# 0215Arthur/Pytorch_News_Recommender

Measured on AMD Instinct MI355X. Metric: users/sec (train step) NRMS MIND-small hist=50 cand=5, higher is better.
Workload: dtype f16 (MFMA inputs and saved activations; fp32 accumulate, softmax, loss, master weights and Adam); 1 GPU; configs[1] shapes: NRMS(nrms_v0) train step, 512 users/GPU, hist=50, cand=5, title_len=30, d=300, h=10, q=200, V=45800, dropout=0.2, Adam(lr=1e-3); users_per_gpu=512, global_batch=512, parallelism=dp1, precision=fp16, resident_batches=32

## Files before the change

pytorch_news_recommender_amd/csrc/fused16.h:

```cpp
#pragma once
#include "gemm.h"

namespace nrms {

typedef _Float16 h8 __attribute__((ext_vector_type(8)));
typedef _Float16 h4 __attribute__((ext_vector_type(4)));
typedef _Float16 h2 __attribute__((ext_vector_type(2)));

__device__ __forceinline__ f32x16 mfma32h(const h8& a, const h8& b, const f32x16& c) {
    return __builtin_amdgcn_mfma_f32_32x32x16_f16(a, b, c, 0, 0, 0);
}

__device__ __forceinline__ h8 acc_frag(const f32x16& x, int s) {
    h8 r;
#pragma unroll
    for (int j = 0; j < 8; ++j) r[j] = (_Float16)x[8 * s + j];
    return r;
}

__device__ __forceinline__ int p16_pos(int fpad) {
    const int b = fpad >> 4, t = fpad & 15;
    const int hh = (t >> 2) & 1, j = ((t >> 3) << 2) | (t & 3);
    return 16 * b + 8 * hh + j;
}

#ifdef NRMS_F16_EXPERIMENTS
#define F16_DBG(flags, bit) ((flags) & (bit))
#else
#define F16_DBG(flags, bit) 0
#endif

constexpr int F16_WAVES = 4;
constexpr int F16_THREADS = 64 * F16_WAVES;
constexpr int F16_KS = 20;
constexpr int F16_CS = 20;
constexpr int F16_QT = 7;
constexpr int F16_KP = 16 * F16_KS, F16_DP = 16 * F16_CS, F16_QP = 32 * F16_QT;
constexpr int F16_PITCH = (F16_KP + 8) * 2;
constexpr int F16_SLOT = 32 * F16_PITCH;
constexpr int F16_RC = F16_KP / 8;
static_assert(F16_KP == F16_DP, "one tile geometry for the head tiles and the additive tiles");
constexpr int F16_STG = (32 * F16_RC + F16_THREADS - 1) / F16_THREADS;
constexpr bool F16_STG_EXACT = 32 * F16_RC == F16_STG * F16_THREADS;

__device__ __forceinline__ long frag_off(long seq_block, int c16, int s, int l32, int hh) {
    return (seq_block * c16 + s) * 512 + l32 * 16 + 8 * hh;
}

struct TileRing {
    char* smem;
    const _Float16* src;
    int n_tiles, tid, l32, hh;
    int dbg;
    h8 stg[F16_STG];
    __device__ __forceinline__ void load(int n) {
        if (n >= n_tiles) return;
        if (F16_DBG(dbg, 1)) return;
        const char* t = reinterpret_cast<const char*>(src) + (long)n * (32 * F16_KP * 2);
        const unsigned off = (unsigned)tid * 16u;
#pragma unroll
        for (int i = 0; i < F16_STG; ++i)
            if (F16_STG_EXACT || i + 1 < F16_STG || tid + F16_THREADS * i < 32 * F16_RC)
                stg[i] = *reinterpret_cast<const h8*>(t + (long)F16_THREADS * 16 * i + off);
    }
    __device__ __forceinline__ void store(int n) {
        if (n >= n_tiles) return;
        if (F16_DBG(dbg, 1)) return;
        char* dst = smem + (n % 3) * F16_SLOT;
#pragma unroll
        for (int i = 0; i < F16_STG; ++i) {
            const int c = tid + F16_THREADS * i;
            if (F16_STG_EXACT || i + 1 < F16_STG || c < 32 * F16_RC) {
                const int row = c / F16_RC, col = c - row * F16_RC;
                *reinterpret_cast<h8*>(dst + row * F16_PITCH + col * 16) = stg[i];
            }
        }
    }
    __device__ __forceinline__ h8 frag(int n, int s) const {
        return *reinterpret_cast<const h8*>(smem + (n % 3) * F16_SLOT + l32 * F16_PITCH + (16 * s + 8 * hh) * 2);
    }
};

constexpr int F16_SLOT_DMA = 32 * F16_KP * 2;
static_assert(F16_SLOT_DMA == 5 * F16_WAVES * 1024, "five 1-KiB DMA pieces per wave and tile");
template <int SLOTS>
struct TileRingDMA {
    static constexpr int AHEAD = SLOTS - 1;
    char* smem;
    const _Float16* src;
    int n_tiles, wave, lane, l32, hh;
    __device__ __forceinline__ void load(int n) {
        if (n >= n_tiles) return;
        const char* g = reinterpret_cast<const char*>(src) + (long)n * F16_SLOT_DMA + wave * 1024 + lane * 16;
        char* l = smem + (n % SLOTS) * F16_SLOT_DMA + wave * 1024;
#pragma unroll
        for (int i = 0; i < 5; ++i)
            __builtin_amdgcn_global_load_lds((const __attribute__((address_space(1))) void*)(g + i * (F16_WAVES * 1024)),
                                             (__attribute__((address_space(3))) void*)(l + i * (F16_WAVES * 1024)), 16, 0, 0);
    }
    __device__ __forceinline__ void load_piece(int n, int i) {
        if (n >= n_tiles) return;
        const char* g = reinterpret_cast<const char*>(src) + (long)n * F16_SLOT_DMA + wave * 1024 + lane * 16 + i * (F16_WAVES * 1024);
        char* l = smem + (n % SLOTS) * F16_SLOT_DMA + wave * 1024 + i * (F16_WAVES * 1024);
        __builtin_amdgcn_global_load_lds((const __attribute__((address_space(1))) void*)g, (__attribute__((address_space(3))) void*)l, 16, 0, 0);
    }
    __device__ __forceinline__ void load_group(int n, int g) {
        if (SLOTS == 3) { load_piece(n, g); return; }
        if (g == 0) { load_piece(n, 0); load_piece(n, 1); }
        if (g == 1) { load_piece(n, 2); load_piece(n, 3); }
        if (g == 2) load_piece(n, 4);
    }
    __device__ __forceinline__ void load_at(int step, int tile) {
        const char* g = reinterpret_cast<const char*>(src) + (long)tile * F16_SLOT_DMA + wave * 1024 + lane * 16;
        char* l = smem + (step % SLOTS) * F16_SLOT_DMA + wave * 1024;
#pragma unroll
        for (int i = 0; i < 5; ++i)
            __builtin_amdgcn_global_load_lds((const __attribute__((address_space(1))) void*)(g + i * (F16_WAVES * 1024)),
                                             (__attribute__((address_space(3))) void*)(l + i * (F16_WAVES * 1024)), 16, 0, 0);
    }
    __device__ __forceinline__ void load_piece_at(int step, int tile, int i) {
        const char* g = reinterpret_cast<const char*>(src) + (long)tile * F16_SLOT_DMA + wave * 1024 + lane * 16 + i * (F16_WAVES * 1024);
        char* l = smem + (step % SLOTS) * F16_SLOT_DMA + wave * 1024 + i * (F16_WAVES * 1024);
        __builtin_amdgcn_global_load_lds((const __attribute__((address_space(1))) void*)g, (__attribute__((address_space(3))) void*)l, 16, 0, 0);
    }
    __device__ __forceinline__ void store(int) {}
    template <int YOUNGER = 0>
    __device__ __forceinline__ void step_barrier(int n) {
        static_assert(YOUNGER == 0 || YOUNGER == 2 || YOUNGER == 4 || YOUNGER == 8, "add the immediate below");
        if (SLOTS == 3 && n + 2 < n_tiles) {
            if (YOUNGER == 0) __asm__ volatile("s_waitcnt vmcnt(5)" ::: "memory");
            if (YOUNGER == 2) __asm__ volatile("s_waitcnt vmcnt(7)" ::: "memory");
            if (YOUNGER == 4) __asm__ volatile("s_waitcnt vmcnt(9)" ::: "memory");
            if (YOUNGER == 8) __asm__ volatile("s_waitcnt vmcnt(13)" ::: "memory");
        } else {
            __asm__ volatile("s_waitcnt vmcnt(0)" ::: "memory");
        }
        __asm__ volatile("s_waitcnt lgkmcnt(0)\n\ts_barrier" ::: "memory");
    }
    __device__ __forceinline__ h8 frag(int n, int s) const {
        return *reinterpret_cast<const h8*>(smem + (n % SLOTS) * F16_SLOT_DMA + ((2 * s + hh) * 32 + l32) * 16);
    }
};
__host__ __device__ __forceinline__ int dma_tile_pos(int r, int k) { return (((k >> 4) * 2 + ((k >> 3) & 1)) * 32 + r) * 8 + (k & 7); }

struct NoPrefetch { __device__ __forceinline__ void operator()(int) const {} };
template <bool W_IS_A, class Ring, int NS, class Between = NoPrefetch>
__device__ __forceinline__ void tile_mma(f32x16& acc, const Ring& ring, int n, const h8 (&op)[NS], Between between = Between()) {
    static_assert(NS % 4 == 0, "k-steps in groups of 4");
    h8 wa[4], wb[4];
#pragma unroll
    for (int i = 0; i < 4; ++i) wa[i] = ring.frag(n, i);
#pragma unroll
    for (int g = 0; g < NS / 4; ++g) {
        if (g + 1 < NS / 4) {
#pragma unroll
            for (int i = 0; i < 4; ++i) {
                if (g & 1) wa[i] = ring.frag(n, 4 * (g + 1) + i);
                else wb[i] = ring.frag(n, 4 * (g + 1) + i);
            }
        }
#pragma unroll
        for (int i = 0; i < 4; ++i) {
            const h8& w = (g & 1) ? wb[i] : wa[i];
            acc = W_IS_A ? mfma32h(w, op[4 * g + i], acc) : mfma32h(op[4 * g + i], w, acc);
        }
        between(g);
        __builtin_amdgcn_sched_barrier(0);
    }
}

__device__ __forceinline__ f32x16 rows_of(const float* v, int hh) {
    f32x16 r;
#pragma unroll
    for (int g = 0; g < 4; ++g) {
        const f32x4 bb = *reinterpret_cast<const f32x4*>(v + 8 * g + 4 * hh);
#pragma unroll
        for (int e = 0; e < 4; ++e) r[4 * g + e] = bb[e];
    }
    return r;
}
__device__ __forceinline__ f32x16 zero16() {
    f32x16 r;
#pragma unroll
    for (int i = 0; i < 16; ++i) r[i] = 0.f;
    return r;
}


}
```

pytorch_news_recommender_amd/csrc/fused16.hip:

```cpp
#include <stdlib.h>

#include "fused16.h"

namespace nrms {

struct Fwd16Args {
    int n_seq, S, d, h, dk, q;
    const _Float16* x16;
    const int* pos;
    const int* n_rows;
    const int64_t* ids;
    const int* order;
    const int* order_cnt;
    const _Float16* wtiles;
    const float* bqkv32;
    const float* badd32;
    const float* qv32;
    _Float16* ctx16;
    _Float16* t16;
    float* w;
    float* out;
    Dropout drop;
    int dbg;
};

#ifndef F16_FWD_SLOTS
#define F16_FWD_SLOTS 3
#endif
constexpr int F16_FWD_WGS = F16_FWD_SLOTS == 2 ? 3 : 2;
template <bool TRAIN, int SB>
__global__ __launch_bounds__(F16_THREADS, SB == 1 ? F16_FWD_WGS : 1) void fused_fwd16_kernel(Fwd16Args a) {
    extern __shared__ __attribute__((aligned(16))) char smem[];
    const int tid = threadIdx.x, lane = tid & 63;
    const int wave = __builtin_amdgcn_readfirstlane(tid >> 6);
    const int l32 = lane & 31, hh = lane >> 5;
    const int S = a.S;
    constexpr int KP = F16_KP, DP = F16_DP;
    const int n_head_tiles = 3 * a.h;

    int slot_id = blockIdx.x * F16_WAVES + wave;
    bool valid = slot_id < a.n_seq;
    int seq = slot_id;
    if (a.order != nullptr) {
        const int n_ne = a.order_cnt[0], n_e = a.order_cnt[1];
        const int g_ne = (n_ne + F16_WAVES - 1) / F16_WAVES;
        if ((int)blockIdx.x < g_ne) { valid = slot_id < n_ne; seq = valid ? a.order[slot_id] : 0; }
        else {
            slot_id -= g_ne * F16_WAVES;
            valid = slot_id < n_e;
            seq = valid ? a.order[a.n_seq + slot_id] : 0;
        }
    }
    if (!valid) seq = 0;
    const long tok0 = (long)seq * S;
    bool tok_ok[SB];
#pragma unroll
    for (int b = 0; b < SB; ++b) tok_ok[b] = valid && 32 * b + l32 < S;
    bool empty = false;
    if (SB == 1 && a.ids != nullptr && valid) {
        const bool is_pad = lane < S ? a.ids[tok0 + lane] == 0 : true;
        empty = __ballot(is_pad) == ~0ull;
    }
    const bool live = valid && !empty;
    const bool skip_heads = __syncthreads_and(live ? 0 : 1) != 0;
    const int n_begin = skip_heads ? n_head_tiles : 0;

    using Ring = TileRingDMA<SB == 1 ? F16_FWD_SLOTS : 3>;
    constexpr int AH = Ring::AHEAD;
    Ring ring;
    ring.smem = smem; ring.src = a.wtiles; ring.n_tiles = n_head_tiles + F16_QT; ring.wave = wave; ring.lane = lane; ring.l32 = l32; ring.hh = hh;
#pragma unroll
    for (int i = 0; i < AH; ++i) ring.load(n_begin + i);
    float* addv = reinterpret_cast<float*>(smem + (SB == 1 ? F16_FWD_SLOTS : 3) * F16_SLOT_DMA);
    for (int i = tid; i < 2 * F16_QP; i += F16_THREADS) addv[i] = i < F16_QP ? a.badd32[i] : a.qv32[i - F16_QP];

    h8 xf[SB][F16_KS];
#pragma unroll
    for (int b = 0; b < SB; ++b) {
        long row = -1;
        if (tok_ok[b] && !empty) {
            row = a.pos != nullptr ? (long)a.pos[tok0 + 32 * b + l32] : tok0 + 32 * b + l32;
            if (row < 0) row = *a.n_rows;
        }
        const _Float16* xr = a.x16 + (row < 0 ? 0 : row) * KP + 8 * hh;
#pragma unroll
        for (int s = 0; s < F16_KS; ++s) xf[b][s] = *reinterpret_cast<const h8*>(xr + 16 * s);
        if (row < 0) {
#pragma unroll
            for (int s = 0; s < F16_KS; ++s) xf[b][s] = h8{0, 0, 0, 0, 0, 0, 0, 0};
        }
    }
    __builtin_amdgcn_s_waitcnt(0x0F70);
    __asm__ volatile("s_waitcnt lgkmcnt(0)\n\ts_barrier" ::: "memory");

    int n = n_begin;
#pragma unroll 1
    for (int head = 0; head < a.h; ++head) {
        f32x16 ct[SB];
        if (!skip_heads) {
            f32x16 qt[SB], kt[SB], vv[SB];
            auto pre = [&](int g) { ring.load_group(n + AH, g); };
            if (!live) ring.load(n + AH);
#pragma unroll
            for (int b = 0; b < SB; ++b) {
                qt[b] = zero16();
                if (live) { if (b == 0) tile_mma<true>(qt[b], ring, n, xf[b], pre); else tile_mma<true>(qt[b], ring, n, xf[b]); }
            }
            ring.step_barrier(n);
            ++n;
            if (!live) ring.load(n + AH);
#pragma unroll
            for (int b = 0; b < SB; ++b) {
                kt[b] = zero16();
                if (live) { if (b == 0) tile_mma<true>(kt[b], ring, n, xf[b], pre); else tile_mma<true>(kt[b], ring, n, xf[b]); }
            }
            ring.step_barrier(n);
            ++n;
            if (!live) ring.load(n + AH);
#pragma unroll
            for (int b = 0; b < SB; ++b) {
                vv[b] = zero16();
                if (live) { if (b == 0) tile_mma<false>(vv[b], ring, n, xf[b], pre); else tile_mma<false>(vv[b], ring, n, xf[b]); }
            }
            if (live) {
#pragma unroll
                for (int ib = 0; ib < SB; ++ib) {
                    f32x16 st[SB];
                    float m = -3.0e38f;
#pragma unroll
                    for (int jb = 0; jb < SB; ++jb) {
                        st[jb] = mfma32h(acc_frag(kt[jb], 0), acc_frag(qt[ib], 0), zero16());
                        st[jb] = mfma32h(acc_frag(kt[jb], 1), acc_frag(qt[ib], 1), st[jb]);
#pragma unroll
                        for (int r = 0; r < 16; ++r) {
                            st[jb][r] = 32 * jb + crow32(r, hh) < S ? st[jb][r] : -3.0e38f;
                            m = fmaxf(m, st[jb][r]);
                        }
                    }
                    m = fmaxf(m, __shfl_xor(m, 32, 64));
                    float sum = 0.f;
#pragma unroll
                    for (int jb = 0; jb < SB; ++jb)
#pragma unroll
                        for (int r = 0; r < 16; ++r) {
                            const float p = 32 * jb + crow32(r, hh) < S ? __expf(st[jb][r] - m) : 0.f;
                            st[jb][r] = p;
                            sum += p;
                        }
                    sum += __shfl_xor(sum, 32, 64);
                    const float inv = 1.0f / sum;
                    ct[ib] = zero16();
#pragma unroll
                    for (int jb = 0; jb < SB; ++jb) {
#pragma unroll
                        for (int r = 0; r < 16; ++r) st[jb][r] *= inv;
                        ct[ib] = mfma32h(acc_frag(vv[jb], 0), acc_frag(st[jb], 0), ct[ib]);
                        ct[ib] = mfma32h(acc_frag(vv[jb], 1), acc_frag(st[jb], 1), ct[ib]);
                    }
                }
            }
        }
        if (!live) {
#pragma unroll
            for (int b = 0; b < SB; ++b) ct[b] = rows_of(a.bqkv32 + (3 * head + 2) * 32, hh);
        }
#pragma unroll
        for (int b = 0; b < SB; ++b) {
            if (a.drop.thresh != 0u) {
#pragma unroll
                for (int c = 0; c < 2; ++c) {
                    const uint64_t e0 = (uint64_t)(tok0 + 32 * b + l32) * (uint64_t)DP + (uint64_t)(head * 32 + 16 * c + 8 * hh);
                    float sc[8];
                    dropout_scale8(a.drop.seed, 1u, e0 >> 3, a.drop.thresh16, a.drop.inv_keep, sc);
#pragma unroll
                    for (int e = 0; e < 8; ++e) ct[b][8 * c + e] *= sc[e];
                }
            }
            if (valid && !F16_DBG(a.dbg, 8)) {
                const h8 z = {0, 0, 0, 0, 0, 0, 0, 0};
                _Float16* dst = a.ctx16 + frag_off((long)seq * SB + b, F16_CS, 2 * head, l32, hh);
                *reinterpret_cast<h8*>(dst) = tok_ok[b] ? acc_frag(ct[b], 0) : z;
                *reinterpret_cast<h8*>(dst + 512) = tok_ok[b] ? acc_frag(ct[b], 1) : z;
            }
        }
        if (!skip_heads) {
            ring.step_barrier(n);
            ++n;
        }
    }
#pragma unroll
    for (int b = 0; b < SB; ++b) {
        if (valid) {
            for (int head = a.h; head < F16_CS / 2; ++head) {
                _Float16* dst = a.ctx16 + frag_off((long)seq * SB + b, F16_CS, 2 * head, l32, hh);
                *reinterpret_cast<h8*>(dst) = h8{0, 0, 0, 0, 0, 0, 0, 0};
                *reinterpret_cast<h8*>(dst + 512) = h8{0, 0, 0, 0, 0, 0, 0, 0};
            }
        }
    }

    __asm__ volatile("s_waitcnt vmcnt(0)" ::: "memory");
    h8 cf[SB][F16_CS];
#pragma unroll
    for (int b = 0; b < SB; ++b) {
        const _Float16* src = a.ctx16 + frag_off((long)seq * SB + b, F16_CS, 0, l32, hh);
#pragma unroll
        for (int s = 0; s < F16_CS; ++s) cf[b][s] = *reinterpret_cast<const h8*>(src + (F16_DBG(a.dbg, 16) ? 0 : 512 * s));
    }
    float score[SB];
#pragma unroll
    for (int b = 0; b < SB; ++b) score[b] = 0.f;
#pragma unroll 1
    for (int t = 0; t < F16_QT; ++t) {
        const f32x16 ba = rows_of(addv + 32 * t, hh), qq = rows_of(addv + F16_QP + 32 * t, hh);
        __builtin_amdgcn_sched_barrier(0);
        auto pre2 = [&](int g) { ring.load_group(n + AH, g); };
        if (!valid) ring.load(n + AH);
#pragma unroll
        for (int b = 0; b < SB; ++b) {
            f32x16 tt = zero16();
            if (valid) { if (b == 0) tile_mma<true>(tt, ring, n, cf[b], pre2); else tile_mma<true>(tt, ring, n, cf[b]); }
#pragma unroll
            for (int g = 0; g < 4; ++g) {
                h4 th;
#pragma unroll
                for (int e = 0; e < 4; ++e) {
                    const float ex = __builtin_amdgcn_exp2f(fmaf(tt[4 * g + e], 2.885390082f, ba[4 * g + e]));
                    const float v = fmaf(-2.0f, __builtin_amdgcn_rcpf(ex + 1.0f), 1.0f);
                    score[b] += qq[4 * g + e] * v;
                    th[e] = (_Float16)v;
                }
                if (TRAIN && valid && !F16_DBG(a.dbg, 4)) {
                    if (!tok_ok[b]) th = h4{0, 0, 0, 0};
                    *reinterpret_cast<h4*>(a.t16 + ((((long)seq * SB + b) * (F16_QP / 16) + 2 * t + (g >> 1)) * 32 + l32) * 16 +
                                           8 * (g & 1) + 4 * hh) = th;
                }
            }
        }
        ring.step_barrier(n);
        ++n;
    }
    float mx = -3.0e38f;
#pragma unroll
    for (int b = 0; b < SB; ++b) {
        score[b] += __shfl_xor(score[b], 32, 64);
        score[b] = 32 * b + l32 < S ? score[b] : -3.0e38f;
        mx = fmaxf(mx, score[b]);
    }
#pragma unroll
    for (int o = 16; o > 0; o >>= 1) mx = fmaxf(mx, __shfl_xor(mx, o, 64));
    float es = 0.f, wgt[SB];
#pragma unroll
    for (int b = 0; b < SB; ++b) {
        wgt[b] = 32 * b + l32 < S ? __expf(score[b] - mx) : 0.f;
        es += wgt[b];
    }
#pragma unroll
    for (int o = 16; o > 0; o >>= 1) es += __shfl_xor(es, o, 64);
#pragma unroll
    for (int b = 0; b < SB; ++b) {
        wgt[b] /= es;
        if (TRAIN && a.w != nullptr && tok_ok[b] && hh == 0) a.w[tok0 + 32 * b + l32] = wgt[b];
    }

    if (valid) {
        h8 sel[2];
#pragma unroll
        for (int s2 = 0; s2 < 2; ++s2)
#pragma unroll
            for (int j = 0; j < 8; ++j) sel[s2][j] = (_Float16)(l32 == 16 * s2 + 8 * hh + j ? 1.0f : 0.0f);
        float wrow[SB][16];
#pragma unroll
        for (int b = 0; b < SB; ++b)
#pragma unroll
            for (int r = 0; r < 16; ++r) wrow[b][r] = __shfl(wgt[b], crow32(r, hh), 64);
#pragma unroll
        for (int p = 0; p < F16_CS / 2; ++p) {
            float acc = 0.f;
#pragma unroll
            for (int b = 0; b < SB; ++b) {
                f32x16 dd = mfma32h(cf[b][2 * p], sel[0], zero16());
                dd = mfma32h(cf[b][2 * p + 1], sel[1], dd);
#pragma unroll
                for (int r = 0; r < 16; ++r) acc += wrow[b][r] * dd[r];
            }
            acc += __shfl_xor(acc, 32, 64);
            const int n = l32, f = 16 * (n >> 4) + 8 * ((n & 7) >> 2) + 4 * ((n >> 3) & 1) + (n & 3);
            if (hh == 0 && f < a.dk && p < a.h) a.out[(long)seq * a.d + p * a.dk + f] = acc;
        }
    }
}

template <bool TRAIN>
__global__ __launch_bounds__(F16_THREADS, F16_FWD_WGS) void fused_fwd16p_kernel(Fwd16Args a) {
    extern __shared__ __attribute__((aligned(16))) char smem[];
    const int tid = threadIdx.x, lane = tid & 63;
    const int wave = __builtin_amdgcn_readfirstlane(tid >> 6);
    const int l32 = lane & 31, hh = lane >> 5;
    const int S = a.S;
    constexpr int KP = F16_KP, DP = F16_DP;
    const int n_head_tiles = 3 * a.h;
    constexpr float NEG = -3.0e38f;

    const int n_long = a.order_cnt[0], n_e = a.order_cnt[1], n_short = a.order_cnt[2];
    const int g_pair = (n_short + 2 * F16_WAVES - 1) / (2 * F16_WAVES);
    const int g_long = (n_long + F16_WAVES - 1) / F16_WAVES, g_e = (n_e + F16_WAVES - 1) / F16_WAVES;
    const int blk = blockIdx.x;
    if (blk >= g_pair + g_long + g_e) return;
    const bool pair = blk < g_pair, skip_heads = blk >= g_pair + g_long;
    const int NT = pair ? 2 : 1;
    int seq[2] = {0, 0};
    bool val[2] = {false, false};
    if (pair) {
        const int p0 = 2 * (blk * F16_WAVES + wave);
#pragma unroll
        for (int i = 0; i < 2; ++i) { val[i] = p0 + i < n_short; seq[i] = val[i] ? a.order[2 * (long)a.n_seq + p0 + i] : 0; }
    } else if (!skip_heads) {
        const int sl = (blk - g_pair) * F16_WAVES + wave;
        val[0] = sl < n_long; seq[0] = val[0] ? a.order[sl] : 0;
    } else {
        const int sl = (blk - g_pair - g_long) * F16_WAVES + wave;
        val[0] = sl < n_e; seq[0] = val[0] ? a.order[(long)a.n_seq + sl] : 0;
    }
    long tok0[2];
    int nlive[2];
#pragma unroll
    for (int i = 0; i < 2; ++i) {
        tok0[i] = (long)seq[i] * S;
        nlive[i] = 0;
        if (pair && val[i]) nlive[i] = __popcll(__ballot(lane < S && a.ids[tok0[i] + lane] != 0));
    }

    const int myp = pair ? (l32 >> 4) : 0, myr = pair ? (l32 & 15) : l32;
    const int myn = myp ? nlive[1] : nlive[0];
    const bool myval = myp ? val[1] : val[0];
    long xrow = -1;
    if (!skip_heads && myval) {
        const long t0 = myp ? tok0[1] : tok0[0];
        if (pair) {
            if (myr < myn) xrow = a.pos[t0 + myr];
            else if (myr == myn && myn < S) xrow = *a.n_rows;
        } else if (myr < S) {
            xrow = a.pos[t0 + myr];
            if (xrow < 0) xrow = *a.n_rows;
        }
    }
    f32x16 kbias;
#pragma unroll
    for (int r = 0; r < 16; ++r) {
        const int j = crow32(r, hh);
        float bsv;
        if (pair) {
            const int jr = j & 15;
            const float lm = __logf((float)max(S - myn, 1));
            bsv = (j >> 4) != myp ? NEG : (jr < myn ? 0.f : ((jr == myn && myn < S) ? lm : NEG));
        } else {
            bsv = j < S ? 0.f : NEG;
        }
        kbias[r] = bsv;
    }
    int src_lane[2];
#pragma unroll
    for (int i = 0; i < 2; ++i) src_lane[i] = 4 * (16 * i + min(l32, nlive[i]) + 32 * hh);
    bool tok_ok[2];
#pragma unroll
    for (int i = 0; i < 2; ++i) tok_ok[i] = val[i] && l32 < S;

    const int n_head_steps = skip_heads ? 0 : n_head_tiles;
    const int n_steps = n_head_steps + F16_QT * NT;
    auto tile_at = [&](int step) { return step < n_head_steps ? step : n_head_tiles + (step - n_head_steps) % F16_QT; };
    using Ring = TileRingDMA<F16_FWD_SLOTS>;
    constexpr int AH = Ring::AHEAD;
    Ring ring;
    ring.smem = smem; ring.src = a.wtiles; ring.n_tiles = n_steps; ring.wave = wave; ring.lane = lane; ring.l32 = l32; ring.hh = hh;
#pragma unroll
    for (int i = 0; i < AH; ++i) ring.load_at(i, tile_at(i));
    float* addv = reinterpret_cast<float*>(smem + F16_FWD_SLOTS * F16_SLOT_DMA);
    for (int i = tid; i < 2 * F16_QP; i += F16_THREADS) addv[i] = i < F16_QP ? a.badd32[i] : a.qv32[i - F16_QP];

    h8 xf[F16_KS];
    {
        const _Float16* xr = a.x16 + (xrow < 0 ? 0 : xrow) * KP + 8 * hh;
#pragma unroll
        for (int s = 0; s < F16_KS; ++s) xf[s] = *reinterpret_cast<const h8*>(xr + 16 * s);
        if (xrow < 0) {
#pragma unroll
            for (int s = 0; s < F16_KS; ++s) xf[s] = h8{0, 0, 0, 0, 0, 0, 0, 0};
        }
    }
    __builtin_amdgcn_s_waitcnt(0x0F70);
    __asm__ volatile("s_waitcnt lgkmcnt(0)\n\ts_barrier" ::: "memory");

    const bool any_live = val[0] || val[1];
    int n = 0;
#pragma unroll 1
    for (int head = 0; head < a.h; ++head) {
        f32x16 ct;
        if (!skip_heads) {
            f32x16 qt = zero16(), kt = zero16(), vv = zero16();
            auto pre = [&](int g) { if (n + AH < n_steps) ring.load_piece_at(n + AH, tile_at(n + AH), g); };
            if (!any_live && n + AH < n_steps) ring.load_at(n + AH, tile_at(n + AH));
            if (any_live) tile_mma<true>(qt, ring, n, xf, pre);
            ring.step_barrier(n);
            ++n;
            if (!any_live && n + AH < n_steps) ring.load_at(n + AH, tile_at(n + AH));
            if (any_live) tile_mma<true>(kt, ring, n, xf, pre);
            ring.step_barrier(n);
            ++n;
            if (!any_live && n + AH < n_steps) ring.load_at(n + AH, tile_at(n + AH));
            if (any_live) tile_mma<false>(vv, ring, n, xf, pre);
            if (any_live) {
                f32x16 st = mfma32h(acc_frag(kt, 0), acc_frag(qt, 0), zero16());
                st = mfma32h(acc_frag(kt, 1), acc_frag(qt, 1), st);
                float m = NEG;
#pragma unroll
                for (int r = 0; r < 16; ++r) { st[r] += kbias[r]; m = fmaxf(m, st[r]); }
                m = fmaxf(m, __shfl_xor(m, 32, 64));
                float sum = 0.f;
#pragma unroll
                for (int r = 0; r < 16; ++r) { st[r] = __expf(st[r] - m); sum += st[r]; }
                sum += __shfl_xor(sum, 32, 64);
                const float inv = 1.0f / sum;
#pragma unroll
                for (int r = 0; r < 16; ++r) st[r] *= inv;
                ct = mfma32h(acc_frag(vv, 0), acc_frag(st, 0), zero16());
                ct = mfma32h(acc_frag(vv, 1), acc_frag(st, 1), ct);
            } else {
                ct = zero16();
            }
        } else {
            ct = rows_of(a.bqkv32 + (3 * head + 2) * 32, hh);
        }
#pragma unroll
        for (int i = 0; i < 2; ++i) {
            if (i < NT) {
                f32x16 cx = ct;
                if (pair) {
#pragma unroll
                    for (int r = 0; r < 16; ++r)
                        cx[r] = __int_as_float(__builtin_amdgcn_ds_bpermute(src_lane[i], __float_as_int(ct[r])));
                }
                if (a.drop.thresh != 0u) {
#pragma unroll
                    for (int c = 0; c < 2; ++c) {
                        const uint64_t e0 = (uint64_t)(tok0[i] + l32) * (uint64_t)DP + (uint64_t)(head * 32 + 16 * c + 8 * hh);
                        float sc[8];
                        dropout_scale8(a.drop.seed, 1u, e0 >> 3, a.drop.thresh16, a.drop.inv_keep, sc);
#pragma unroll
                        for (int e = 0; e < 8; ++e) cx[8 * c + e] *= sc[e];
                    }
                }
                if (val[i]) {
                    const h8 z = {0, 0, 0, 0, 0, 0, 0, 0};
                    _Float16* dst = a.ctx16 + frag_off((long)seq[i], F16_CS, 2 * head, l32, hh);
                    *reinterpret_cast<h8*>(dst) = tok_ok[i] ? acc_frag(cx, 0) : z;
                    *reinterpret_cast<h8*>(dst + 512) = tok_ok[i] ? acc_frag(cx, 1) : z;
                }
            }
        }
        if (!skip_heads) {
            ring.step_barrier(n);
            ++n;
        }
    }
#pragma unroll
    for (int i = 0; i < 2; ++i) {
        if (i < NT && val[i]) {
            for (int head = a.h; head < F16_CS / 2; ++head) {
                _Float16* dst = a.ctx16 + frag_off((long)seq[i], F16_CS, 2 * head, l32, hh);
                *reinterpret_cast<h8*>(dst) = h8{0, 0, 0, 0, 0, 0, 0, 0};
                *reinterpret_cast<h8*>(dst + 512) = h8{0, 0, 0, 0, 0, 0, 0, 0};
            }
        }
    }

#pragma unroll 1
    for (int i = 0; i < NT; ++i) {
        const bool valid = i ? val[1] : val[0];
        const bool tok = i ? tok_ok[1] : tok_ok[0];
        const int sq = i ? seq[1] : seq[0];
        const long t0 = i ? tok0[1] : tok0[0];
        __asm__ volatile("s_waitcnt vmcnt(0)" ::: "memory");
        h8 cf[F16_CS];
        {
            const _Float16* src = a.ctx16 + frag_off((long)sq, F16_CS, 0, l32, hh);
#pragma unroll
            for (int s = 0; s < F16_CS; ++s) cf[s] = *reinterpret_cast<const h8*>(src + 512 * s);
        }
        float score = 0.f;
#pragma unroll 1
        for (int t = 0; t < F16_QT; ++t) {
            const f32x16 ba = rows_of(addv + 32 * t, hh), qq = rows_of(addv + F16_QP + 32 * t, hh);
            __builtin_amdgcn_sched_barrier(0);
            auto pre2 = [&](int g) { if (n + AH < n_steps) ring.load_piece_at(n + AH, tile_at(n + AH), g); };
            if (!valid && n + AH < n_steps) ring.load_at(n + AH, tile_at(n + AH));
            f32x16 tt = zero16();
            if (valid) tile_mma<true>(tt, ring, n, cf, pre2);
#pragma unroll
            for (int g = 0; g < 4; ++g) {
                h4 th;
#pragma unroll
                for (int e = 0; e < 4; ++e) {
                    const float ex = __builtin_amdgcn_exp2f(fmaf(tt[4 * g + e], 2.885390082f, ba[4 * g + e]));
                    const float v = fmaf(-2.0f, __builtin_amdgcn_rcpf(ex + 1.0f), 1.0f);
                    score += qq[4 * g + e] * v;
                    th[e] = (_Float16)v;
                }
                if (TRAIN && valid) {
                    if (!tok) th = h4{0, 0, 0, 0};
                    *reinterpret_cast<h4*>(a.t16 + (((long)sq * (F16_QP / 16) + 2 * t + (g >> 1)) * 32 + l32) * 16 + 8 * (g & 1) + 4 * hh) = th;
                }
            }
            ring.step_barrier(n);
            ++n;
        }
        score += __shfl_xor(score, 32, 64);
        score = l32 < S ? score : NEG;
        float mx = score;
#pragma unroll
        for (int o = 16; o > 0; o >>= 1) mx = fmaxf(mx, __shfl_xor(mx, o, 64));
        float wgt = l32 < S ? __expf(score - mx) : 0.f;
        float es = wgt;
#pragma unroll
        for (int o = 16; o > 0; o >>= 1) es += __shfl_xor(es, o, 64);
        wgt /= es;
        if (TRAIN && a.w != nullptr && tok && hh == 0) a.w[t0 + l32] = wgt;
        if (valid) {
            h8 sel[2];
#pragma unroll
            for (int s2 = 0; s2 < 2; ++s2)
#pragma unroll
                for (int j = 0; j < 8; ++j) sel[s2][j] = (_Float16)(l32 == 16 * s2 + 8 * hh + j ? 1.0f : 0.0f);
            float wrow[16];
#pragma unroll
            for (int r = 0; r < 16; ++r) wrow[r] = __shfl(wgt, crow32(r, hh), 64);
#pragma unroll
            for (int p = 0; p < F16_CS / 2; ++p) {
                f32x16 dd = mfma32h(cf[2 * p], sel[0], zero16());
                dd = mfma32h(cf[2 * p + 1], sel[1], dd);
                float acc = 0.f;
#pragma unroll
                for (int r = 0; r < 16; ++r) acc += wrow[r] * dd[r];
                acc += __shfl_xor(acc, 32, 64);
                const int nn = l32, f = 16 * (nn >> 4) + 8 * ((nn & 7) >> 2) + 4 * ((nn >> 3) & 1) + (nn & 3);
                if (hh == 0 && f < a.dk && p < a.h) a.out[(long)sq * a.d + p * a.dk + f] = acc;
            }
        }
    }
}

struct Prep16Args {
    int d, h, dk, q, KP, DP, QP;
    const float* w_qkv;
    const float* b_qkv;
    const float* w_add;
    const float* b_add;
    const float* q_vec;
    _Float16* wqkv16;
    float* bqkv32;
    _Float16* wadd16;
    float* badd32;
    float* qv32;
};

__global__ __launch_bounds__(256) void prep16_kernel(Prep16Args a) {
    const float qscale = 1.0f / sqrtf((float)a.dk);
    const long n1 = (long)3 * a.h * 32 * a.KP, n2 = (long)a.QP * a.DP, n3 = (long)3 * a.h * 32, n4 = a.QP;
    const long total = n1 + n2 + n3 + 2 * n4;
    for (long i = (long)blockIdx.x * blockDim.x + threadIdx.x; i < total; i += (long)gridDim.x * blockDim.x) {
        if (i < n1) {
            const int k = (int)(i % a.KP);
            const long r = i / a.KP;
            const int f = (int)(r & 31), tile = (int)(r >> 5), head = tile / 3, which = tile - 3 * head;
            float v = 0.f;
            if (f < a.dk && k < a.d) v = a.w_qkv[((long)which * a.d + head * a.dk + f) * a.d + k] * (which == 0 ? qscale : 1.0f);
            if (f < a.dk && k == a.d) v = a.b_qkv[which * a.d + head * a.dk + f] * (which == 0 ? qscale : 1.0f);
            a.wqkv16[(long)tile * 32 * a.KP + dma_tile_pos(f, k)] = (_Float16)v;
        } else if (i < n1 + n2) {
            const long j = i - n1;
            const int p = (int)(j % a.DP), qq = (int)(j / a.DP);
            const int b16 = p >> 4, t = p & 15, hh = t >> 3, jj = t & 7;
            const int fpad = 16 * b16 + 8 * (jj >> 2) + 4 * hh + (jj & 3);
            const int head = fpad >> 5, f = fpad & 31;
            float v = 0.f;
            if (qq < a.q && f < a.dk) v = a.w_add[(long)qq * a.d + head * a.dk + f];
            a.wadd16[(long)(qq >> 5) * 32 * a.DP + dma_tile_pos(qq & 31, p)] = (_Float16)v;
        } else if (i < n1 + n2 + n3) {
            const long j = i - n1 - n2;
            const int f = (int)(j & 31), tile = (int)(j >> 5), head = tile / 3, which = tile - 3 * head;
            float v = 0.f;
            if (f < a.dk) v = a.b_qkv[which * a.d + head * a.dk + f] * (which == 0 ? qscale : 1.0f);
            a.bqkv32[j] = v;
        } else if (i < n1 + n2 + n3 + n4) {
            const long j = i - n1 - n2 - n3;
            a.badd32[j] = j < a.q ? a.b_add[j] * 2.885390082f : 0.f;
        } else {
            const long j = i - n1 - n2 - n3 - n4;
            a.qv32[j] = j < a.q ? a.q_vec[j] : 0.f;
        }
    }
}

template <int NCLS, bool PLACE>
__global__ __launch_bounds__(256) void title_order_kernel(int n_seq, int S, const int64_t* ids, int* order, int* cnt) {
    __shared__ int flag[256];
    __shared__ int wcount[4][NCLS], base[NCLS], part[4][NCLS];
    const int lane = threadIdx.x & 63, wave = threadIdx.x >> 6;
    const int t0 = blockIdx.x * 256;
#pragma unroll 1
    for (int r = 0; r < 4; ++r) {
        int64_t v[16];
#pragma unroll
        for (int i = 0; i < 16; ++i) {
            const int t = min(t0 + wave * 64 + r * 16 + i, n_seq - 1);
            v[i] = ids[(long)t * S + min(lane, S - 1)];
        }
#pragma unroll
        for (int i = 0; i < 16; ++i) {
            const int t = t0 + wave * 64 + r * 16 + i;
            const unsigned long long livemask = __ballot(lane < S && v[i] != 0);
            int cls = livemask == 0ull ? 1 : 0;
            if (NCLS == 3 && livemask != 0ull) {
                const int n = __popcll(livemask);
                if (n <= 15 && livemask == (1ull << n) - 1ull) cls = 2;
            }
            if (lane == 0) flag[wave * 64 + r * 16 + i] = t < n_seq ? cls : -1;
        }
    }
    __syncthreads();
    const int f = flag[threadIdx.x];
    const unsigned long long below = (1ull << lane) - 1ull;
    int rank = 0;
#pragma unroll
    for (int c = 0; c < NCLS; ++c) {
        const unsigned long long m = __ballot(f == c);
        if (f == c) rank = __popcll(m & below);
        if (lane == 0) wcount[wave][c] = __popcll(m);
    }
    if (PLACE) {
        int s[NCLS];
#pragma unroll
        for (int c = 0; c < NCLS; ++c) s[c] = 0;
        for (int b = threadIdx.x; b < (int)blockIdx.x; b += 256)
#pragma unroll
            for (int c = 0; c < NCLS; ++c) s[c] += cnt[NCLS + NCLS * b + c];
#pragma unroll
        for (int c = 0; c < NCLS; ++c) {
#pragma unroll
            for (int o = 32; o > 0; o >>= 1) s[c] += __shfl_xor(s[c], o, 64);
            if (lane == 0) part[wave][c] = s[c];
        }
    }
    __syncthreads();
    if (threadIdx.x < NCLS) {
        const int c = threadIdx.x;
        const int mine = wcount[0][c] + wcount[1][c] + wcount[2][c] + wcount[3][c];
        if (!PLACE) cnt[NCLS + NCLS * blockIdx.x + c] = mine;
        else {
            base[c] = part[0][c] + part[1][c] + part[2][c] + part[3][c];
            if (blockIdx.x == gridDim.x - 1) cnt[c] = base[c] + mine;
        }
    }
    if (!PLACE) return;
    __syncthreads();
    if (f >= 0) {
        for (int w = 0; w < wave; ++w) rank += wcount[w][f];
        order[(long)f * n_seq + base[f] + rank] = t0 + threadIdx.x;
    }
}

size_t title_order_cnt_ints(int n_seq) { return 3 + 3 * (size_t)cdiv(n_seq > 0 ? n_seq : 1, 256); }

int launch_title_order(int n_seq, int S, const int64_t* ids, int* order, int* cnt, hipStream_t stream, int n_classes) {
    if (n_seq <= 0) return NRMS_OK;
    TimingScope ts("title_order", stream);
    const dim3 grid(cdiv(n_seq, 256));
    if (n_classes == 3) {
        hipLaunchKernelGGL((title_order_kernel<3, false>), grid, dim3(256), 0, stream, n_seq, S, ids, order, cnt);
        hipLaunchKernelGGL((title_order_kernel<3, true>), grid, dim3(256), 0, stream, n_seq, S, ids, order, cnt);
    } else {
        hipLaunchKernelGGL((title_order_kernel<2, false>), grid, dim3(256), 0, stream, n_seq, S, ids, order, cnt);
        hipLaunchKernelGGL((title_order_kernel<2, true>), grid, dim3(256), 0, stream, n_seq, S, ids, order, cnt);
    }
    return check_launch("title_order");
}

__global__ __launch_bounds__(256) void gather16_kernel(unsigned d4, unsigned kp4, long M, const int64_t* ids, const int* live,
                                                       const int* n_live, const float* table, Dropout drop, _Float16* x16) {
    const unsigned rows = live != nullptr ? (unsigned)(*n_live) : (unsigned)M;
    const unsigned total = (rows + (live != nullptr ? 1u : 0u)) * kp4;
    const unsigned stride = gridDim.x * blockDim.x;
    for (unsigned i = blockIdx.x * blockDim.x + threadIdx.x; i < total; i += stride) {
        const unsigned r = i / kp4, c4 = i - r * kp4;
        h4 o = {0, 0, 0, 0};
        if (c4 == d4) o[0] = (_Float16)1.0f;
        if (r >= rows) { *reinterpret_cast<h4*>(x16 + (long)i * 4) = o; continue; }
        const long t = live != nullptr ? (long)live[r] : (long)r;
        if (c4 < d4) {
            f32x4 v = *reinterpret_cast<const f32x4*>(table + ids[t] * (long)(4 * d4) + 4 * c4);
            if (drop.thresh != 0u) v *= dropout_scale4(drop.seed, 0u, (uint64_t)(t * d4 + c4), drop.thresh, drop.inv_keep);
#pragma unroll
            for (int e = 0; e < 4; ++e) o[e] = (_Float16)v[e];
        }
        *reinterpret_cast<h4*>(x16 + (long)i * 4) = o;
    }
}

__global__ __launch_bounds__(256) void cast16_kernel(unsigned d4, unsigned kp4, long M, const float* x, _Float16* x16) {
    const unsigned total = (unsigned)M * kp4;
    for (unsigned i = blockIdx.x * blockDim.x + threadIdx.x; i < total; i += gridDim.x * blockDim.x) {
        const unsigned r = i / kp4, c4 = i - r * kp4;
        h4 o = {0, 0, 0, 0};
        if (c4 == d4) o[0] = (_Float16)1.0f;
        if (c4 < d4) {
            const f32x4 v = *reinterpret_cast<const f32x4*>(x + ((long)r * d4 + c4) * 4);
#pragma unroll
            for (int e = 0; e < 4; ++e) o[e] = (_Float16)v[e];
        }
        *reinterpret_cast<h4*>(x16 + (long)i * 4) = o;
    }
}

bool fused16_supported(int S, int d, int h, int q, const char** why) {
    const int dk = d / h;
    const char* w = nullptr;
    if (S > 64) w = "seq_len <= 64";
    else if (d > F16_KP - 4) w = "d_model <= 316";
    else if (dk > 32) w = "d_k <= 32";
    else if (32 * h > F16_DP) w = "n_heads <= 10";
    else if (q > F16_QP) w = "q_dim <= 224";
    if (why) *why = w;
    return w == nullptr;
}

Fused16Layout fused16_layout(int d, int h, int q) {
    Fused16Layout L;
    L.KP = F16_KP;
    L.DP = F16_DP;
    L.QP = F16_QP;
    size_t off = 0;
    auto take = [&](size_t bytes) { size_t o = off; off = (off + bytes + 255) / 256 * 256; return o; };
    L.wqkv16 = take((size_t)3 * h * 32 * L.KP * 2 + (size_t)L.QP * L.DP * 2);
    L.wadd16 = L.wqkv16 + (size_t)3 * h * 32 * L.KP * 2;
    L.bqkv32 = take((size_t)3 * h * 32 * 4);
    L.badd32 = take((size_t)L.QP * 4);
    L.qv32 = take((size_t)L.QP * 4);
    L.total = off;
    return L;
}

int launch_prep16(int d, int h, int q, const float* w_qkv, const float* b_qkv, const float* w_add, const float* b_add,
                  const float* q_vec, void* planes, hipStream_t stream) {
    const Fused16Layout L = fused16_layout(d, h, q);
    char* base = (char*)planes;
    Prep16Args a{};
    a.d = d; a.h = h; a.dk = d / h; a.q = q; a.KP = L.KP; a.DP = L.DP; a.QP = L.QP;
    a.w_qkv = w_qkv; a.b_qkv = b_qkv; a.w_add = w_add; a.b_add = b_add; a.q_vec = q_vec;
    a.wqkv16 = (_Float16*)(base + L.wqkv16); a.wadd16 = (_Float16*)(base + L.wadd16);
    a.bqkv32 = (float*)(base + L.bqkv32); a.badd32 = (float*)(base + L.badd32); a.qv32 = (float*)(base + L.qv32);
    const long total = (long)3 * h * 32 * L.KP + (long)L.QP * L.DP + 3 * h * 32 + 2 * L.QP;
    TimingScope ts("prep16", stream);
    hipLaunchKernelGGL(prep16_kernel, dim3(cdiv(total, 256)), dim3(256), 0, stream, a);
    return check_launch("prep16");
}

int launch_gather16(long M, int d, int KP, const int64_t* ids, const int* live, const int* n_live, const float* table,
                    const Dropout& drop, void* x16, hipStream_t stream) {
    if (M <= 0) return NRMS_OK;
    if ((M + 1) * (KP / 4) >= (1L << 32)) { set_error("gather16: index overflow"); return NRMS_EINVAL; }
    int blocks = cdiv((M + 1) * (KP / 4), 256);
    if (blocks > 256 * 16) blocks = 256 * 16;
    TimingScope ts("gather_dropout", stream);
    hipLaunchKernelGGL(gather16_kernel, dim3(blocks), dim3(256), 0, stream, (unsigned)(d / 4), (unsigned)(KP / 4), M, ids, live,
                       n_live, table, drop, (_Float16*)x16);
    return check_launch("gather16");
}

int launch_cast16(long M, int d, int KP, const float* x, void* x16, hipStream_t stream) {
    if (M <= 0) return NRMS_OK;
    if (M * (KP / 4) >= (1L << 32)) { set_error("cast16: index overflow"); return NRMS_EINVAL; }
    int blocks = cdiv(M * (KP / 4), 256);
    if (blocks > 256 * 16) blocks = 256 * 16;
    TimingScope ts("cast16", stream);
    hipLaunchKernelGGL(cast16_kernel, dim3(blocks), dim3(256), 0, stream, (unsigned)(d / 4), (unsigned)(KP / 4), M, x, (_Float16*)x16);
    return check_launch("cast16");
}

int launch_fused_fwd16(const Fused16Fwd& f, hipStream_t stream) {
    if (f.n_seq <= 0) return NRMS_OK;
    const Fused16Layout L = fused16_layout(f.d, f.h, f.q);
    const char* base = (const char*)f.planes;
    Fwd16Args a{};
    a.n_seq = f.n_seq; a.S = f.S; a.d = f.d; a.h = f.h; a.dk = f.d / f.h; a.q = f.q;
    a.x16 = (const _Float16*)f.x16; a.pos = f.pos; a.n_rows = f.n_rows; a.ids = f.ids; a.order = f.order; a.order_cnt = f.order_cnt;
    a.wtiles = (const _Float16*)(base + L.wqkv16); a.bqkv32 = (const float*)(base + L.bqkv32);
    a.badd32 = (const float*)(base + L.badd32); a.qv32 = (const float*)(base + L.qv32);
    a.ctx16 = (_Float16*)f.ctx16; a.t16 = (_Float16*)f.t16; a.w = f.w; a.out = f.out; a.drop = f.drop;
    const bool train = f.t16 != nullptr, two = f.S > 32;
    const size_t lds = (size_t)(two ? 3 : F16_FWD_SLOTS) * F16_SLOT_DMA + (size_t)2 * F16_QP * 4;
    a.dbg = 0;
#ifdef NRMS_F16_EXPERIMENTS
    { const char* e = getenv("NRMS_F16_DBG"); a.dbg = e ? atoi(e) : 0; }
#endif
    const bool paired = !two && f.order != nullptr && f.pos != nullptr && f.ids != nullptr;
    if (!paired) { a.order = nullptr; a.order_cnt = nullptr; }
    const void* fn = paired ? (train ? (const void*)fused_fwd16p_kernel<true> : (const void*)fused_fwd16p_kernel<false>)
                   : two ? (train ? (const void*)fused_fwd16_kernel<true, 2> : (const void*)fused_fwd16_kernel<false, 2>)
                         : (train ? (const void*)fused_fwd16_kernel<true, 1> : (const void*)fused_fwd16_kernel<false, 1>);
    const hipError_t e = hipFuncSetAttribute(fn, hipFuncAttributeMaxDynamicSharedMemorySize, (int)lds);
    if (e != hipSuccess) { set_error("fused_fwd16: hipFuncSetAttribute: %s", hipGetErrorString(e)); return NRMS_ELAUNCH; }
    TimingScope ts(two ? "fused64_fwd16" : "fused_fwd16", stream);
    const dim3 grid(cdiv(f.n_seq, F16_WAVES) + (f.order != nullptr ? 3 : 0));
    if (paired) {
        if (train) hipLaunchKernelGGL((fused_fwd16p_kernel<true>), grid, dim3(F16_THREADS), lds, stream, a);
        else hipLaunchKernelGGL((fused_fwd16p_kernel<false>), grid, dim3(F16_THREADS), lds, stream, a);
    } else if (two) {
        if (train) hipLaunchKernelGGL((fused_fwd16_kernel<true, 2>), grid, dim3(F16_THREADS), lds, stream, a);
        else hipLaunchKernelGGL((fused_fwd16_kernel<false, 2>), grid, dim3(F16_THREADS), lds, stream, a);
    } else {
        if (train) hipLaunchKernelGGL((fused_fwd16_kernel<true, 1>), grid, dim3(F16_THREADS), lds, stream, a);
        else hipLaunchKernelGGL((fused_fwd16_kernel<false, 1>), grid, dim3(F16_THREADS), lds, stream, a);
    }
    return check_launch("fused_fwd16");
}

}
```

Baseline: 167,900 users/s.

## Split empty-history blocks into a dedicated closed-form forward path

Blocks that handle sequences whose heads are skipped now run a separate device function. It builds the context fragments straight in registers from the value bias times the dropout scale, writes them to ctx16, and runs the additive pooling. Before, these blocks went through the general kernel path, reading the bias rows and writing then reloading ctx16 through global memory. The pooling loop is moved into a shared helper, and the skip_heads branches are removed from the main path, which cuts branching and register pressure for the normal blocks. The risk is that the closed-form fragments no longer match the earlier write and reload path exactly, and the extra kernel branch adds code size.

```diff
diff --git a/pytorch_news_recommender_amd/csrc/fused16.h b/pytorch_news_recommender_amd/csrc/fused16.h
--- a/pytorch_news_recommender_amd/csrc/fused16.h
+++ b/pytorch_news_recommender_amd/csrc/fused16.h
@@ -16,6 +16,12 @@
 #pragma unroll
     for (int j = 0; j < 8; ++j) r[j] = (_Float16)x[8 * s + j];
     return r;
+}
+
+__device__ __forceinline__ _Float16 closed_ctx16(float b_v, float scale) {
+    float p = b_v * scale;
+    __asm__ volatile("" : "+v"(p));
+    return (_Float16)p;
 }
 
 __device__ __forceinline__ int p16_pos(int fpad) {
diff --git a/pytorch_news_recommender_amd/csrc/fused16.hip b/pytorch_news_recommender_amd/csrc/fused16.hip
--- a/pytorch_news_recommender_amd/csrc/fused16.hip
+++ b/pytorch_news_recommender_amd/csrc/fused16.hip
@@ -291,6 +291,129 @@
     }
 }
 
+template <bool TRAIN, class Ring, class TileAt>
+__device__ __forceinline__ void fwd16p_additive_pool(const Fwd16Args& a, Ring& ring, int& n, int n_steps, TileAt tile_at, const float* addv,
+                                                     const h8 (&cf)[F16_CS], bool valid, bool tok, int sq, long t0, int l32, int hh) {
+    constexpr int AH = Ring::AHEAD;
+    constexpr float NEG = -3.0e38f;
+    const int S = a.S;
+    float score = 0.f;
+#pragma unroll 1
+    for (int t = 0; t < F16_QT; ++t) {
+        const f32x16 ba = rows_of(addv + 32 * t, hh), qq = rows_of(addv + F16_QP + 32 * t, hh);
+        __builtin_amdgcn_sched_barrier(0);
+        auto pre2 = [&](int g) { if (n + AH < n_steps) ring.load_piece_at(n + AH, tile_at(n + AH), g); };
+        if (!valid && n + AH < n_steps) ring.load_at(n + AH, tile_at(n + AH));
+        f32x16 tt = zero16();
+        if (valid) tile_mma<true>(tt, ring, n, cf, pre2);
+#pragma unroll
+        for (int g = 0; g < 4; ++g) {
+            h4 th;
+#pragma unroll
+            for (int e = 0; e < 4; ++e) {
+                const float ex = __builtin_amdgcn_exp2f(fmaf(tt[4 * g + e], 2.885390082f, ba[4 * g + e]));
+                const float v = fmaf(-2.0f, __builtin_amdgcn_rcpf(ex + 1.0f), 1.0f);
+                score += qq[4 * g + e] * v;
+                th[e] = (_Float16)v;
+            }
+            if (TRAIN && valid) {
+                if (!tok) th = h4{0, 0, 0, 0};
+                *reinterpret_cast<h4*>(a.t16 + (((long)sq * (F16_QP / 16) + 2 * t + (g >> 1)) * 32 + l32) * 16 + 8 * (g & 1) + 4 * hh) = th;
+            }
+        }
+        ring.step_barrier(n);
+        ++n;
+    }
+    score += __shfl_xor(score, 32, 64);
+    score = l32 < S ? score : NEG;
+    float mx = score;
+#pragma unroll
+    for (int o = 16; o > 0; o >>= 1) mx = fmaxf(mx, __shfl_xor(mx, o, 64));
+    float wgt = l32 < S ? __expf(score - mx) : 0.f;
+    float es = wgt;
+#pragma unroll
+    for (int o = 16; o > 0; o >>= 1) es += __shfl_xor(es, o, 64);
+    wgt /= es;
+    if (TRAIN && a.w != nullptr && tok && hh == 0) a.w[t0 + l32] = wgt;
+    if (valid) {
+        h8 sel[2];
+#pragma unroll
+        for (int s2 = 0; s2 < 2; ++s2)
+#pragma unroll
+            for (int j = 0; j < 8; ++j) sel[s2][j] = (_Float16)(l32 == 16 * s2 + 8 * hh + j ? 1.0f : 0.0f);
+        float wrow[16];
+#pragma unroll
+        for (int r = 0; r < 16; ++r) wrow[r] = __shfl(wgt, crow32(r, hh), 64);
+#pragma unroll
+        for (int p = 0; p < F16_CS / 2; ++p) {
+            f32x16 dd = mfma32h(cf[2 * p], sel[0], zero16());
+            dd = mfma32h(cf[2 * p + 1], sel[1], dd);
+            float acc = 0.f;
+#pragma unroll
+            for (int r = 0; r < 16; ++r) acc += wrow[r] * dd[r];
+            acc += __shfl_xor(acc, 32, 64);
+            const int nn = l32, f = 16 * (nn >> 4) + 8 * ((nn & 7) >> 2) + 4 * ((nn >> 3) & 1) + (nn & 3);
+            if (hh == 0 && f < a.dk && p < a.h) a.out[(long)sq * a.d + p * a.dk + f] = acc;
+        }
+    }
+}
+
+template <bool TRAIN>
+__device__ __forceinline__ void fwd16p_closed(const Fwd16Args& a, char* smem, int first_slot, int n_e) {
+    const int tid = threadIdx.x, lane = tid & 63;
+    const int wave = __builtin_amdgcn_readfirstlane(tid >> 6);
+    const int l32 = lane & 31, hh = lane >> 5;
+    constexpr int DP = F16_DP;
+    const int sl = first_slot + wave;
+    const bool valid = sl < n_e;
+    const int sq = valid ? a.order[(long)a.n_seq + sl] : 0;
+    const long t0 = (long)sq * a.S;
+    const bool tok = valid && l32 < a.S;
+
+    const int first_tile = 3 * a.h;
+    auto tile_at = [&](int step) { return first_tile + step; };
+    using Ring = TileRingDMA<F16_FWD_SLOTS>;
+    constexpr int AH = Ring::AHEAD;
+    Ring ring;
+    ring.smem = smem; ring.src = a.wtiles; ring.n_tiles = F16_QT; ring.wave = wave; ring.lane = lane; ring.l32 = l32; ring.hh = hh;
+#pragma unroll
+    for (int i = 0; i < AH; ++i) ring.load_at(i, tile_at(i));
+    float* addv = reinterpret_cast<float*>(smem + F16_FWD_SLOTS * F16_SLOT_DMA);
+    for (int i = tid; i < 2 * F16_QP; i += F16_THREADS) addv[i] = i < F16_QP ? a.badd32[i] : a.qv32[i - F16_QP];
+
+    h8 cf[F16_CS];
+#pragma unroll
+    for (int head = 0; head < F16_CS / 2; ++head) {
+#pragma unroll
+        for (int c = 0; c < 2; ++c) {
+            h8 fr = {0, 0, 0, 0, 0, 0, 0, 0};
+            if (head < a.h && tok) {
+                const float* bv = a.bqkv32 + (3 * head + 2) * 32 + 16 * c + 4 * hh;
+                const f32x4 b0 = *reinterpret_cast<const f32x4*>(bv), b1 = *reinterpret_cast<const f32x4*>(bv + 8);
+                float sc[8];
+#pragma unroll
+                for (int e = 0; e < 8; ++e) sc[e] = 1.0f;
+                if (a.drop.thresh != 0u) {
+                    const uint64_t e0 = (uint64_t)(t0 + l32) * (uint64_t)DP + (uint64_t)(head * 32 + 16 * c + 8 * hh);
+                    dropout_scale8(a.drop.seed, 1u, e0 >> 3, a.drop.thresh16, a.drop.inv_keep, sc);
+                }
+#pragma unroll
+                for (int e = 0; e < 8; ++e) fr[e] = closed_ctx16(e < 4 ? b0[e & 3] : b1[e & 3], sc[e]);
+            }
+            cf[2 * head + c] = fr;
+        }
+    }
+    __builtin_amdgcn_s_waitcnt(0x0F70);
+    __asm__ volatile("s_waitcnt lgkmcnt(0)\n\ts_barrier" ::: "memory");
+    int n = 0;
+    fwd16p_additive_pool<TRAIN>(a, ring, n, F16_QT, tile_at, addv, cf, valid, tok, sq, t0, l32, hh);
+    if (valid) {
+        _Float16* dst = a.ctx16 + frag_off((long)sq, F16_CS, 0, l32, hh);
+#pragma unroll
+        for (int s = 0; s < F16_CS; ++s) *reinterpret_cast<h8*>(dst + 512 * s) = cf[s];
+    }
+}
+
 template <bool TRAIN>
 __global__ __launch_bounds__(F16_THREADS, F16_FWD_WGS) void fused_fwd16p_kernel(Fwd16Args a) {
     extern __shared__ __attribute__((aligned(16))) char smem[];
@@ -307,7 +430,11 @@
     const int g_long = (n_long + F16_WAVES - 1) / F16_WAVES, g_e = (n_e + F16_WAVES - 1) / F16_WAVES;
     const int blk = blockIdx.x;
     if (blk >= g_pair + g_long + g_e) return;
-    const bool pair = blk < g_pair, skip_heads = blk >= g_pair + g_long;
+    if (blk >= g_pair + g_long) {
+        fwd16p_closed<TRAIN>(a, smem, (blk - g_pair - g_long) * F16_WAVES, n_e);
+        return;
+    }
+    const bool pair = blk < g_pair;
     const int NT = pair ? 2 : 1;
     int seq[2] = {0, 0};
     bool val[2] = {false, false};
@@ -315,12 +442,9 @@
         const int p0 = 2 * (blk * F16_WAVES + wave);
 #pragma unroll
         for (int i = 0; i < 2; ++i) { val[i] = p0 + i < n_short; seq[i] = val[i] ? a.order[2 * (long)a.n_seq + p0 + i] : 0; }
-    } else if (!skip_heads) {
+    } else {
         const int sl = (blk - g_pair) * F16_WAVES + wave;
         val[0] = sl < n_long; seq[0] = val[0] ? a.order[sl] : 0;
-    } else {
-        const int sl = (blk - g_pair - g_long) * F16_WAVES + wave;
-        val[0] = sl < n_e; seq[0] = val[0] ? a.order[(long)a.n_seq + sl] : 0;
     }
     long tok0[2];
     int nlive[2];
@@ -335,7 +459,7 @@
     const int myn = myp ? nlive[1] : nlive[0];
     const bool myval = myp ? val[1] : val[0];
     long xrow = -1;
-    if (!skip_heads && myval) {
+    if (myval) {
         const long t0 = myp ? tok0[1] : tok0[0];
         if (pair) {
             if (myr < myn) xrow = a.pos[t0 + myr];
@@ -366,9 +490,8 @@
 #pragma unroll
     for (int i = 0; i < 2; ++i) tok_ok[i] = val[i] && l32 < S;
 
-    const int n_head_steps = skip_heads ? 0 : n_head_tiles;
-    const int n_steps = n_head_steps + F16_QT * NT;
-    auto tile_at = [&](int step) { return step < n_head_steps ? step : n_head_tiles + (step - n_head_steps) % F16_QT; };
+    const int n_steps = n_head_tiles + F16_QT * NT;
+    auto tile_at = [&](int step) { return step < n_head_tiles ? step : n_head_tiles + (step - n_head_tiles) % F16_QT; };
     using Ring = TileRingDMA<F16_FWD_SLOTS>;
     constexpr int AH = Ring::AHEAD;
     Ring ring;
@@ -396,40 +519,36 @@
 #pragma unroll 1
     for (int head = 0; head < a.h; ++head) {
         f32x16 ct;
-        if (!skip_heads) {
-            f32x16 qt = zero16(), kt = zero16(), vv = zero16();
-            auto pre = [&](int g) { if (n + AH < n_steps) ring.load_piece_at(n + AH, tile_at(n + AH), g); };
-            if (!any_live && n + AH < n_steps) ring.load_at(n + AH, tile_at(n + AH));
-            if (any_live) tile_mma<true>(qt, ring, n, xf, pre);
-            ring.step_barrier(n);
-            ++n;
-            if (!any_live && n + AH < n_steps) ring.load_at(n + AH, tile_at(n + AH));
-            if (any_live) tile_mma<true>(kt, ring, n, xf, pre);
-            ring.step_barrier(n);
-            ++n;
-            if (!any_live && n + AH < n_steps) ring.load_at(n + AH, tile_at(n + AH));
-            if (any_live) tile_mma<false>(vv, ring, n, xf, pre);
-            if (any_live) {
-                f32x16 st = mfma32h(acc_frag(kt, 0), acc_frag(qt, 0), zero16());
-                st = mfma32h(acc_frag(kt, 1), acc_frag(qt, 1), st);
-                float m = NEG;
-#pragma unroll
-                for (int r = 0; r < 16; ++r) { st[r] += kbias[r]; m = fmaxf(m, st[r]); }
-                m = fmaxf(m, __shfl_xor(m, 32, 64));
-                float sum = 0.f;
-#pragma unroll
-                for (int r = 0; r < 16; ++r) { st[r] = __expf(st[r] - m); sum += st[r]; }
-                sum += __shfl_xor(sum, 32, 64);
-                const float inv = 1.0f / sum;
-#pragma unroll
-                for (int r = 0; r < 16; ++r) st[r] *= inv;
-                ct = mfma32h(acc_frag(vv, 0), acc_frag(st, 0), zero16());
-                ct = mfma32h(acc_frag(vv, 1), acc_frag(st, 1), ct);
-            } else {
-                ct = zero16();
-            }
+        f32x16 qt = zero16(), kt = zero16(), vv = zero16();
+        auto pre = [&](int g) { if (n + AH < n_steps) ring.load_piece_at(n + AH, tile_at(n + AH), g); };
+        if (!any_live && n + AH < n_steps) ring.load_at(n + AH, tile_at(n + AH));
+        if (any_live) tile_mma<true>(qt, ring, n, xf, pre);
+        ring.step_barrier(n);
+        ++n;
+        if (!any_live && n + AH < n_steps) ring.load_at(n + AH, tile_at(n + AH));
+        if (any_live) tile_mma<true>(kt, ring, n, xf, pre);
+        ring.step_barrier(n);
+        ++n;
+        if (!any_live && n + AH < n_steps) ring.load_at(n + AH, tile_at(n + AH));
+        if (any_live) tile_mma<false>(vv, ring, n, xf, pre);
+        if (any_live) {
+            f32x16 st = mfma32h(acc_frag(kt, 0), acc_frag(qt, 0), zero16());
+            st = mfma32h(acc_frag(kt, 1), acc_frag(qt, 1), st);
+            float m = NEG;
+#pragma unroll
+            for (int r = 0; r < 16; ++r) { st[r] += kbias[r]; m = fmaxf(m, st[r]); }
+            m = fmaxf(m, __shfl_xor(m, 32, 64));
+            float sum = 0.f;
+#pragma unroll
+            for (int r = 0; r < 16; ++r) { st[r] = __expf(st[r] - m); sum += st[r]; }
+            sum += __shfl_xor(sum, 32, 64);
+            const float inv = 1.0f / sum;
+#pragma unroll
+            for (int r = 0; r < 16; ++r) st[r] *= inv;
+            ct = mfma32h(acc_frag(vv, 0), acc_frag(st, 0), zero16());
+            ct = mfma32h(acc_frag(vv, 1), acc_frag(st, 1), ct);
         } else {
-            ct = rows_of(a.bqkv32 + (3 * head + 2) * 32, hh);
+            ct = zero16();
         }
 #pragma unroll
         for (int i = 0; i < 2; ++i) {
@@ -458,10 +577,8 @@
                 }
             }
         }
-        if (!skip_heads) {
-            ring.step_barrier(n);
-            ++n;
-        }
+        ring.step_barrier(n);
+        ++n;
     }
 #pragma unroll
     for (int i = 0; i < 2; ++i) {
@@ -487,65 +604,7 @@
 #pragma unroll
             for (int s = 0; s < F16_CS; ++s) cf[s] = *reinterpret_cast<const h8*>(src + 512 * s);
         }
-        float score = 0.f;
-#pragma unroll 1
-        for (int t = 0; t < F16_QT; ++t) {
-            const f32x16 ba = rows_of(addv + 32 * t, hh), qq = rows_of(addv + F16_QP + 32 * t, hh);
-            __builtin_amdgcn_sched_barrier(0);
-            auto pre2 = [&](int g) { if (n + AH < n_steps) ring.load_piece_at(n + AH, tile_at(n + AH), g); };
-            if (!valid && n + AH < n_steps) ring.load_at(n + AH, tile_at(n + AH));
-            f32x16 tt = zero16();
-            if (valid) tile_mma<true>(tt, ring, n, cf, pre2);
-#pragma unroll
-            for (int g = 0; g < 4; ++g) {
-                h4 th;
-#pragma unroll
-                for (int e = 0; e < 4; ++e) {
-                    const float ex = __builtin_amdgcn_exp2f(fmaf(tt[4 * g + e], 2.885390082f, ba[4 * g + e]));
-                    const float v = fmaf(-2.0f, __builtin_amdgcn_rcpf(ex + 1.0f), 1.0f);
-                    score += qq[4 * g + e] * v;
-                    th[e] = (_Float16)v;
-                }
-                if (TRAIN && valid) {
-                    if (!tok) th = h4{0, 0, 0, 0};
-                    *reinterpret_cast<h4*>(a.t16 + (((long)sq * (F16_QP / 16) + 2 * t + (g >> 1)) * 32 + l32) * 16 + 8 * (g & 1) + 4 * hh) = th;
-                }
-            }
-            ring.step_barrier(n);
-            ++n;
-        }
-        score += __shfl_xor(score, 32, 64);
-        score = l32 < S ? score : NEG;
-        float mx = score;
-#pragma unroll
-        for (int o = 16; o > 0; o >>= 1) mx = fmaxf(mx, __shfl_xor(mx, o, 64));
-        float wgt = l32 < S ? __expf(score - mx) : 0.f;
-        float es = wgt;
-#pragma unroll
-        for (int o = 16; o > 0; o >>= 1) es += __shfl_xor(es, o, 64);
-        wgt /= es;
-        if (TRAIN && a.w != nullptr && tok && hh == 0) a.w[t0 + l32] = wgt;
-        if (valid) {
-            h8 sel[2];
-#pragma unroll
-            for (int s2 = 0; s2 < 2; ++s2)
-#pragma unroll
-                for (int j = 0; j < 8; ++j) sel[s2][j] = (_Float16)(l32 == 16 * s2 + 8 * hh + j ? 1.0f : 0.0f);
-            float wrow[16];
-#pragma unroll
-            for (int r = 0; r < 16; ++r) wrow[r] = __shfl(wgt, crow32(r, hh), 64);
-#pragma unroll
-            for (int p = 0; p < F16_CS / 2; ++p) {
-                f32x16 dd = mfma32h(cf[2 * p], sel[0], zero16());
-                dd = mfma32h(cf[2 * p + 1], sel[1], dd);
-                float acc = 0.f;
-#pragma unroll
-                for (int r = 0; r < 16; ++r) acc += wrow[r] * dd[r];
-                acc += __shfl_xor(acc, 32, 64);
-                const int nn = l32, f = 16 * (nn >> 4) + 8 * ((nn & 7) >> 2) + 4 * ((nn >> 3) & 1) + (nn & 3);
-                if (hh == 0 && f < a.dk && p < a.h) a.out[(long)sq * a.d + p * a.dk + f] = acc;
-            }
-        }
+        fwd16p_additive_pool<TRAIN>(a, ring, n, n_steps, tile_at, addv, cf, valid, tok, sq, t0, l32, hh);
     }
 }
 
```

Result: faster. 170,600 users/s, median of 6 (+1.6%).
